# Caltech-OCTO/Subzero.jl

Measured on AMD Instinct MI355X. Metric: floe_steps_per_sec, higher is better.
Workload: dtype f64

## Files before the change

### subzero.jl_amd/csrc/sz_api.hip

```cpp
#include <hip/hip_runtime.h>
#include <dlfcn.h>
#include <execinfo.h>
#include <signal.h>
#include <unistd.h>
#include <algorithm>
#include <cmath>
#include <cstdio>
#include <cstring>
#include <string>
#include <vector>

#include "../../include/subzero_hip.h"
#include "sz_kernels.hpp"
#include "sz_pipeline.hpp"
#include "sz_twoway.hpp"
#include "sz_output.hpp"
#include "sz_migrate.hpp"
#include "sz_fracture.hpp"
#include "sz_weld.hpp"
#include "sz_remove_tile.hpp"
#include "sz_fracture_tile.hpp"
#include "sz_weld_tile.hpp"
#include <rocprim/rocprim.hpp>
#include "sz_ctx.hpp"
// ... 168 lines not shown
  (void)hipMemsetAsync(c->S.cell_ovf, 0, ((size_t)c->S.capCells + 1) * sizeof(int), c->stream);
  hipLaunchKernelGGL(sz_k_cell_build, dim3(grid_for(c->S.capM, 256)), dim3(256), 0, c->stream, c->S, 1);
  c->grid_live = true;
}

void world_rings(sz_ctx* c) {
  if (!c->rings_stale) return;
  hipLaunchKernelGGL(sz_k_world_rings, dim3(grid_for(c->S.capM, 256)), dim3(256), 0, c->stream, c->S);
  c->rings_stale = false;
}
void leave_resident(sz_ctx* c) { c->gl_valid = false; c->S.famrec = 0; c->crec_current = false; world_rings(c); }
struct BatchModes {
  sz_ctx* c;
  explicit BatchModes(sz_ctx* c_) : c(c_) { clear(); }
  ~BatchModes() { clear(); }
  BatchModes(const BatchModes&) = delete;
  BatchModes& operator=(const BatchModes&) = delete;
  void clear() {
    State& S = c->S;
    S.step = 0; S.retry_stop = 0; S.stop_on_tags = 0; S.restart_on_tags = 0; S.ginline = 0; S.famrec = 0; S.body_rings = 0;
    S.crec = nullptr; S.facc = nullptr; S.goff = 0; S.gcap = 0; S.pipe = 0;
    c->acc_mode = 0; c->reduce_mode = 0;
  }
};

void use_ghost_list(sz_ctx* c) {
  if (c->gl_valid) return;
  (void)hipMemsetAsync(c->S.cnt + C_NGCAND, 0, 2 * sizeof(int), c->stream);
  c->gl_cur = 0;
  hipLaunchKernelGGL(sz_k_ghost_seed, dim3(grid_for(c->S.capM, 256)), dim3(256), 0, c->stream, c->S, 0);
  c->gl_valid = true;
}
int reseed_inline_ghosts(sz_ctx* c, int slot) {
  HIPCHK(c, hipMemsetAsync(c->S.galloc, 0, 32 * sizeof(unsigned long long), c->stream));
  c->S.gslot = slot;
  hipLaunchKernelGGL(sz_k_ghost_inline_seed, dim3(grid_for(c->S.capM, 256)), dim3(256), 0, c->stream, c->S, slot, c->hostN);
  return SZ_OK;
}
bool ghost_list_wanted(const sz_ctx* c, bool sg) {
  return sg && !c->no_ghost_list && (c->S.any_periodic_ew || c->S.any_periodic_ns) && c->gl_est <= c->gl_max && c->max_ring <= 64;
}

void stage_ghosts(sz_ctx* c, bool in_step = false, bool commit = false, bool use_list = false) {
  State& S = c->S;
  const int nh = in_step && !S.tiled ? c->hostN : -1;
  if (!S.any_periodic_ew && !S.any_periodic_ns) return;
  S.famrec = in_step ? 1 : 0;
  Timed t(c, SZ_K_GHOSTS);
  if (use_list) {
    const int waves = std::min(std::max(2 * c->gl_est + 64, 256), 8192);
    hipLaunchKernelGGL(sz_k_ghost_list, dim3((waves + 3) / 4), dim3(256), 0, c->stream, S, c->gl_cur, 1, nh);
    t.end();
    return;
  }
  const int nb = grid_for(S.capM, SCAN_B, 1 << 20);
  hipLaunchKernelGGL(sz_k_ghost_flag_scan, dim3(nb), dim3(SCAN_B), 0, c->stream, S, in_step ? 1 : 0, commit ? 1 : 0, next_epoch(c), nh);
  hipLaunchKernelGGL(sz_k_ghost_fill, dim3(grid_for(S.capM, 32, 2048)), dim3(256), 0, c->stream, S, commit ? 1 : 0, commit ? 1 : 0, nh);
  if (!in_step) hipLaunchKernelGGL(sz_k_ghost_commit, dim3(1), dim3(64), 0, c->stream, S);
  t.end();
}

int search_grid(const State& T) { return grid_for(T.capM, NB_TPB / NB_G, 8192); }
void launch_search(sz_ctx* c, const State& T, bool elems = false, bool forcing = false) {
  const bool rec = T.crec != nullptr;
  if (forcing) {
    const int nbn = grid_for(T.capM, 256 / NB_G, 8192), nbf = grid_for(T.capM, 256 / FRC_PLAIN, 8192);
    const auto kern = c->precision == 1 ? (rec ? sz_k_neighbors_forcing<2, true> : sz_k_neighbors_forcing<2, false>)
// ... 569 lines not shown
  std::vector<int> tag0;
  DA(frc_remove, S.capM); DA(osign, S.capM); DA(bbx0, S.capM); DA(bbx1, S.capM); DA(bby0, S.capM); DA(bby1, S.capM);
  {
    std::vector<long long> id(M), gid(M, 0);
    std::vector<int> st(M, SZ_ACTIVE), parent(M), gh((size_t)MAX_GHOSTS * M, -1), ngh(M, 0);
    for (int i = 0; i < M; i++) { id[i] = f->id ? f->id[i] : i + 1; if (f->ghost_id) gid[i] = f->ghost_id[i]; if (f->status) st[i] = f->status[i]; parent[i] = i; }
    if (M > N) {
      for (int i = 0; i < N; i++) {
        int n = f->ghost_off[i + 1] - f->ghost_off[i];
        if (n > MAX_GHOSTS) { c->err = "more than 3 ghosts for one parent"; return SZ_E_ARG; }
        ngh[i] = n;
        for (int k = 0; k < n; k++) { int g = f->ghost_idx[f->ghost_off[i] + k]; if (g < N || g >= M) { c->err = "ghost index out of range"; return SZ_E_ARG; } gh[(size_t)i * MAX_GHOSTS + k] = g; parent[g] = i; }
      }
    }
    { std::vector<long long> ok(S.capM); for (int i = 0; i < S.capM; i++) ok[i] = i; H2D(S.okey, ok.data(), S.capM, long long); HIPCHK(c, hipStreamSynchronize(c->stream)); }
    H2D(S.id, id.data(), M, long long); H2D(S.ghost_id, gid.data(), M, long long); H2D(S.status, st.data(), M, int);
    tag0 = st;
    H2D(S.parent, parent.data(), M, int); H2D(S.gh, gh.data(), (size_t)MAX_GHOSTS * M, int); H2D(S.ngh, ngh.data(), M, int);
    HIPCHK(c, hipStreamSynchronize(c->stream));
  }
  DA(voff, S.capM + 1); DA(vxy, S.capV);
  H2D(S.voff, f->vert_off, M + 1, int);
  {
    std::vector<double> xy((size_t)2 * std::max(V, 1));
    for (int k = 0; k < V; k++) { xy[(size_t)2 * k] = f->vx[k]; xy[(size_t)2 * k + 1] = f->vy[k]; }
    H2D(S.vxy, xy.data(), (size_t)2 * V, double); HIPCHK(c, hipStreamSynchronize(c->stream));
  }
  DA(soff, S.capM + 1); DA(sx, NS); DA(sy, NS);
  if (f->sub_off) { H2D(S.soff, f->sub_off, N + 1, int); H2D(S.sx, f->sx, NS, double); H2D(S.sy, f->sy, NS, double); }
  c->max_sub = 0;
  if (f->sub_off) for (int i = 0; i < N; i++) c->max_sub = std::max(c->max_sub, f->sub_off[i + 1] - f->sub_off[i]);
  DA(gplan, S.capM + 1); DA(gscan4, S.capM + 1); DA(gtot4, 4);
  DA(lb_agg, S.capM / 128 + 8); DA(lb_inc, S.capM / 128 + 8); DA(lb_flag, S.capM / 128 + 8);
  DA(gflag, S.capM + 1); DA(gvscan, S.capM + 2); DA(gcand, (size_t)2 * S.capM); DA(galloc, 32); DA(gkeys, (size_t)2 * S.capM); DA(fam, S.capM);
  DA(crec, (size_t)8 * S.capM); c->crec_buf = S.crec; S.crec = nullptr;
  {
    StepSet& B = c->pb[1];
    if ((rc = dalloc(c, &B.vxy, (size_t)S.capV, c->allocs)) || (rc = dalloc(c, &B.crec, (size_t)8 * S.capM, c->allocs)) ||
        (rc = dalloc(c, &B.gh, (size_t)MAX_GHOSTS * S.capM, c->allocs)) || (rc = dalloc(c, &B.ngh, (size_t)S.capM, c->allocs))) return rc;
    HIPCHK(c, hipMemsetAsync(B.gh, 0xff, (size_t)MAX_GHOSTS * S.capM * sizeof(int), c->stream));
    c->gpar = 0;
  }
  DA(facc, (size_t)FX_WORDS * S.capM); c->facc_buf = S.facc; S.facc = nullptr;
  c->maybe_tagged = false;
  if (f->status) for (int i = 0; i < N; i++) if (f->status[i] != SZ_ACTIVE) { c->maybe_tagged = true; break; }
  for (int k = 0; k < 4; k++) if ((rc = dalloc(c, &c->frc_alt[k], (size_t)S.capM, c->allocs))) return rc;
  DA(bounds, 16 + 64 * 4); DA(cell_cnt, S.capCells + 1); DA(cell_ovf, S.capCells + 1); DA(cell_slots, (size_t)S.capCells * CELL_K + 8);
  DA(cell_items, S.capM);
  {
    StepSet& B = c->pb[1];
    if ((rc = dalloc(c, &B.cell_cnt, (size_t)S.capCells + 1, c->allocs)) || (rc = dalloc(c, &B.cell_ovf, (size_t)S.capCells + 1, c->allocs)) ||
        (rc = dalloc(c, &B.cell_slots, (size_t)S.capCells * CELL_K + 8, c->allocs)) || (rc = dalloc(c, &B.cell_items, (size_t)S.capM, c->allocs))) return rc;
  }
  DA(n_out, S.capM + 1); DA(n_in, S.capM + 1); DA(over_stamp, S.capM + 1); DA(over_base, S.capM + 1);
  DA(out_off, S.capM + 2);
  DA(el_off, S.capM + 2); DA(el_floe, S.capElem); DA(el_elem, S.capElem);
  DA(inter_off, S.capM + 2);
  if (!f->sub_off) HIPCHK(c, hipMemsetAsync(S.soff, 0, ((size_t)S.capM + 1) * sizeof(int), c->stream));
  if ((rc = carve_lists(c))) return rc;
  if ((rc = carve_interactions(c))) return rc;
  DA(blk, std::max(S.capCells, std::max(S.capM, 1024)) / SCAN_B + 1024);
  own_set_carved(c);
  DA(tagA, S.capM + 1);
  if (!tag0.empty()) { H2D(S.tagA, tag0.data(), M, int); HIPCHK(c, hipStreamSynchronize(c->stream)); }
  if ((rc = dalloc(c, &c->origin, (size_t)S.capM, c->allocs))) return rc;
  { std::vector<int> o(std::max(M, 1)); for (int i = 0; i < M; i++) o[i] = i; H2D(c->origin, o.data(), M, int); HIPCHK(c, hipStreamSynchronize(c->stream)); }
  DA(stamps, 512 + 8 * 8000);
  trim_pool(c->allocs);
  free_pool(c->comm_allocs);
  int gl_est = N;
  double rmax_max = 0.0;
  if (f->rmax) {
    const double x0 = c->h_vals[3], xf = c->h_vals[2], y0 = c->h_vals[1], yf = c->h_vals[0];
    const bool pew = c->h_kinds[SZ_EAST] == SZ_PERIODIC && c->h_kinds[SZ_WEST] == SZ_PERIODIC;
    const bool pns = c->h_kinds[SZ_NORTH] == SZ_PERIODIC && c->h_kinds[SZ_SOUTH] == SZ_PERIODIC;
    gl_est = 0;
    for (int i = 0; i < N; i++) {
      const double r = f->rmax[i];
      if ((pew && (f->cx[i] - r < x0 || f->cx[i] + r > xf)) || (pns && (f->cy[i] - r < y0 || f->cy[i] + r > yf))) gl_est++;
    }
// ... 561 lines not shown
  p.pipe = pipeline_eligible(c, p, nsteps, flags);
  p.lean = p.coll && lean_wanted(c) && (p.pipe || !c->S.tiled);
  p.first_alone = p.rfree && c->maybe_tagged && p.user_stop && nsteps > 1;
  p.frac = c->frac_kind != SZ_FRAC_OFF && p.user_stop && !p.pipe;
  return p;
}

int step_batch_pipelined(sz_ctx* c, const BatchPlan& plan, int nsteps, int tstep0, int dt, int coupling_dt, int flags, int* h, int* done_out, int* slot_out, bool* rest_out) {
  State& S0 = c->S;
  const int N = c->hostN;
  const bool fam = N <= 40000 && plan.periodic;
  const bool elems = S0.any_domain_work != 0;
  const int q0 = c->gpar;
  auto par = [&](int s) { return (q0 + s) & 1; };
  S0.restart_on_tags = plan.user_stop ? 0 : 1;
  bool lean = plan.lean;
  Clears clr(c);
  clr.add(c->facc_buf, (size_t)FX_WORDS * S0.capM * sizeof(long long));
  clr.add(S0.cnt + C_FRCSTOP, sizeof(int));
  const int callid0 = c->callid; c->callid += nsteps;
  bool first_start = true;
  auto prologue = [&](int s) {
    const int q = par(s);
    pipe_adopt(c, q);
    S0.step = 0; S0.goff = 0; S0.gcap = 0;
    if (!first_start) c->grid_live = false;
    use_static_grid(c);
    const StepSet& O = c->pb[1 - q];
    clr.add(O.cell_cnt, ((size_t)S0.capCells + 1) * sizeof(int));
    clr.add(O.cell_ovf, ((size_t)S0.capCells + 1) * sizeof(int));
    clr.add(c->pb[0].wq, NSEG * 32 * sizeof(int)); clr.add(c->pb[1].wq, NSEG * 32 * sizeof(int));
    clr.add(c->pb[0].ngh, (size_t)S0.capM * sizeof(int));
    clr.add(c->pb[1].ngh, (size_t)S0.capM * sizeof(int));
    clr.add(S0.galloc, 32 * sizeof(unsigned long long));
    clr.launch(c);
    if (!(first_start && c->crec_current))
      for (int b = 0; b < 2; b++) { State T = pipe_state(c, b); T.step = 0; seed_records(c, T, N); }
    first_start = false;
    State T = pipe_state(c, q); T.step = s + 1; T.callid = callid0 + s + 1; T.retry_stop = lean ? 1 : 0;
    if (plan.gi) hipLaunchKernelGGL(sz_k_ghost_inline_seed, dim3(grid_for(S0.capM, 256)), dim3(256), 0, c->stream, T, q, N);
    launch_search(c, T, elems);
  };
  auto launch_L1 = [&](int s, bool make_ghosts) {
    State T = pipe_state(c, par(s)); T.step = s + 1; T.callid = callid0 + s + 1; T.retry_stop = lean ? 1 : 0;
    const PipeAlt A = pipe_alt(c, par(s + 1), make_ghosts ? 1 : 0);
    const bool coupling = coupling_at(flags, coupling_dt, tstep0 + s);
    const bool overlap = coupling && (c->overlap_forcing >= 0 ? c->overlap_forcing != 0 : N > 65536);
    if (overlap) stage_forcing_fork(c, &T);
    if (coupling) c->forcing_where = overlap ? 0 : 2;
    const bool frc = coupling && !overlap;
    launch_narrow_first(c, frc ? narrow_first<1, 1> : narrow_first<0, 1>, T, dt, c->P.ff_max_overlap, c->P.fd_max_overlap, frc, &A, N);
    if (!lean) narrow_largest(c, T, dt, c->P.ff_max_overlap, c->P.fd_max_overlap, 256);
    return overlap;
  };
  auto launch_L2 = [&](int s, bool with_search, bool host_last, bool joined) {
    if (joined) stage_forcing_join(c);
    State T = pipe_state(c, par(s + 1)); T.step = s + 2; T.callid = callid0 + s + 2; T.retry_stop = lean ? 1 : 0;
    const PipeAlt A = pipe_alt(c, par(s), 0);
    const int nbv = grid_for(N, NB_TPB, 1 << 20), nbs = with_search ? search_grid(T) : 0;
    const int nbe = with_search && elems ? grid_for(N, NB_TPB, 1 << 20) : 0;
    const unsigned ep = nbe ? next_epoch(c) : 0u;
    const int am = 1 | 4 | (host_last ? 2 : 0);
    Timed tm(c, SZ_K_INTEGRATE);
    if (fam) hipLaunchKernelGGL((sz_k_vel_search<true>), dim3(nbv + nbs + nbe), dim3(NB_TPB), 0, c->stream, T, c->P, A, dt, coupling_at(flags, coupling_dt, tstep0 + s) ? 1 : 0, nbv, N, am, nbe, ep);
    else hipLaunchKernelGGL((sz_k_vel_search<false>), dim3(nbv + nbs + nbe), dim3(NB_TPB), 0, c->stream, T, c->P, A, dt, coupling_at(flags, coupling_dt, tstep0 + s) ? 1 : 0, nbv, N, am, nbe, ep);
    tm.end();
  };
// ... 902 lines not shown
```

### subzero.jl_amd/csrc/sz_kernels.hpp

```cpp
#pragma once
#include <type_traits>
#include "sz_geom.hpp"
#include "sz_state.hpp"

namespace sz {
using namespace szg;

#define SZ_ACTIVE 1
#define SZ_REMOVE 2
#define SZ_FUSE 3

__device__ __forceinline__ bool stopped(const State& S) {
  const int s = S.cnt[C_STOP], r = S.cnt[C_RETRYSTOP];
  return (s != 0 && S.step > s) || (r != 0 && S.step > r);
}
__device__ __forceinline__ bool stopped_late(const State& S) {
  const int s = S.cnt[C_STOP], r = S.cnt[C_RETRYSTOP];
  return (s != 0 && S.step > s) || (r != 0 && S.step >= r);
}
struct StopRegs { int s, r; };
__device__ __forceinline__ StopRegs stop_load(const State& S) { StopRegs q; q.s = S.cnt[C_STOP]; q.r = S.cnt[C_RETRYSTOP]; return q; }
__device__ __forceinline__ bool stop_test(const State& S, const StopRegs& q) { return (q.s != 0 && S.step > q.s) || (q.r != 0 && S.step > q.r); }
__device__ __forceinline__ bool stop_test_late(const State& S, const StopRegs& q) { return (q.s != 0 && S.step > q.s) || (q.r != 0 && S.step >= q.r); }
__device__ __forceinline__ void loads_issued() { asm volatile("" ::: "memory"); }
__device__ __forceinline__ void request_stop(const State& S) {
  if (S.step > 0 && S.stop_on_tags) S.cnt[C_STOP] = S.step;
}
__device__ __forceinline__ void request_stop_new_tag(const State& S) {
  if (S.step > 0 && (S.stop_on_tags || S.restart_on_tags)) S.cnt[C_STOP] = S.step;
}
__device__ __forceinline__ void capacity_stop(const State& S) {
  if (S.step > 0) S.cnt[C_RETRYSTOP] = S.step;
}

__device__ __forceinline__ int ring_off(const State& S, int i) { return S.body_rings ? S.rb_off[i] : S.voff[i]; }
__device__ __forceinline__ int ring_n(const State& S, int i) { return S.body_rings ? S.rb_n[i] : S.voff[i + 1] - S.voff[i]; }
constexpr float MIX_CIRCLE_MARGIN = 4.0f, MIX_BOX_MARGIN = 2.0f;
__device__ __forceinline__ void rec32_store(const State& S, int i, double cx, double cy, double r, double x0, double x1, double y0, double y1) {
  S.rec32[2 * (size_t)i] = make_float4((float)cx, (float)cy, (float)r, 0.0f);
  S.rec32[2 * (size_t)i + 1] = make_float4((float)x0, (float)x1, (float)y0, (float)y1);
}

constexpr long long CREC_KEYMASK = (1ll << 48) - 1;
__device__ __forceinline__ double crec_okf(long long okey, int nv, int osign) {
  return __longlong_as_double(okey | ((long long)(nv & 255) << 48) | ((long long)(osign < 0 ? 1 : 0) << 56));
}
__device__ __forceinline__ double crec_vp(int voff, int parent, int ngh) {
  return __longlong_as_double((long long)(unsigned)voff | ((long long)parent << 32) | ((long long)ngh << 60));
}
__device__ __forceinline__ void crec_store_all(const State& S, int row, double cx, double cy, double rmax, long long id, long long okey, int nv, int osign,
                                               int voff, int parent, int ngh, double x0, double x1, double y0, double y1, double u, double v, double xi,
                                               double area, double h, long long ghost_id) {
  double2* r = S.crec + (size_t)row * 8;
  r[0] = make_double2(cx, cy); r[1] = make_double2(rmax, __longlong_as_double(id));
  r[2] = make_double2(crec_okf(okey, nv, osign), crec_vp(voff, parent, ngh));
  r[3] = make_double2(x0, x1); r[4] = make_double2(y0, y1); r[5] = make_double2(u, v); r[6] = make_double2(xi, area);
  r[7] = make_double2(h, __longlong_as_double(ghost_id));
// ... 930 lines not shown
    return idx < cnt ? start + idx : -1;
  }
  const int q = nblk / 8, r = nblk % 8;
  return (x < r ? x * (q + 1) : r * (q + 1) + (x - r) * q) + idx;
}


struct Seg { int s, np, ne, n; };
__device__ __forceinline__ int seg_cap(const State& S) { return S.capPairs / NSEG; }
__device__ __forceinline__ Seg seg_of(const State& S, int s) {
  Seg g; g.s = s; g.np = S.wq[s * 32 + 1];
  const int nel = S.cnt[C_NELEM];
  g.ne = nel > s ? (nel - s + NSEG - 1) / NSEG : 0;
  g.n = g.np + g.ne;
  return g;
}
struct Item { int i, j, e, rows, info, ao, na, bo, nb; bool is_pair; };
__device__ __forceinline__ Item item_of(const State& S, const Seg& g, int t) {
  Item it; it.is_pair = t < g.np;
  if (it.is_pair) {
    const int w = g.s * seg_cap(S) + t;
    const int4 k = S.work[2 * (size_t)w], r = S.work[2 * (size_t)w + 1];
    it.info = k.x; it.i = k.y; it.j = k.z; it.e = -1; it.rows = w; it.ao = k.w; it.na = r.x; it.bo = r.y; it.nb = r.z;
  } else {
    const int q = (t - g.np) * NSEG + g.s; it.i = S.el_floe[q]; it.e = S.el_elem[q]; it.j = -1; it.rows = S.capPairs + q; it.info = S.capM * S.maxnb + q;
    it.ao = ring_off(S, it.i); it.na = ring_n(S, it.i); it.bo = S.eoff[it.e]; it.nb = S.eoff[it.e + 1] - it.bo;
  }
  return it;
}

constexpr int NB_G = 16, NB_TPB = 128;
static_assert(NB_G == FX_WORDS, "the neighbour search clears a new row's fixed-point totals with one store per lane");
template <int TPB, bool FAM = true, int NBC = MAXNB, bool REC = false>
__device__ __forceinline__ void neighbors_body(State& S, int bid, int nblk) {
  constexpr int GPB = TPB / NB_G;
  constexpr int NB_POOL = NBC <= 24 ? 96 : (NBC <= 64 ? 224 : 256);
  constexpr int MW = (NBC + 63) / 64;
  static_assert(NB_POOL >= NBC, "the pool is reused for the sorted list of the owned pairs");
  __shared__ int cand[GPB][2][NBC];
  __shared__ long long ckey[GPB][2][NBC];
  __shared__ int cnts[GPB][2];
  using mask_t = typename std::conditional<(NBC <= 32), unsigned, unsigned long long>::type;
  __shared__ mask_t wmask[MW > 1 ? 1 : GPB];
  __shared__ unsigned long long wmaskw[MW > 1 ? GPB : 1][MW];
  __shared__ int pool[GPB][NB_POOL];
  __shared__ int pool2[GPB][NBC > MAXNB ? NB_POOL : 1];
  __shared__ int npool[GPB];
  __shared__ int wbase[GPB + 1];
  __shared__ int cvo[GPB][NBC], cnv[GPB][NBC], svo[GPB][NBC], snv[GPB][NBC];
  __shared__ double kbox[REC ? GPB : 1][4];
  const int gl = threadIdx.x % NB_G, gi = threadIdx.x / NB_G;
  const StopRegs stop = stop_load(S);
  int M = S.cnt[C_M];
  int nfix = 0x7fffffff;
  int nsplit = 0x7fffffff, kshift = 0, lim0 = M, lim1 = M;
  if (S.ginline) {
    const unsigned long long a = S.galloc[S.gslot * 16], poisoned = S.galloc[S.gslot * 16 + 1];
    const int N = S.cnt[C_N]; int G = (int)(a >> 32), V = (int)(a & 0xffffffffull);
    if (REC && S.facc) nfix = N;
    if (poisoned || N + S.goff + G > S.capM || (S.gcap > 0 && G > S.gcap)) { G = 0; V = 0; }
    M = N + G; lim0 = M; lim1 = M;
    if (bid == 0 && threadIdx.x == 0 && !stop_test(S, stop)) { S.cnt[C_M] = M; S.cnt[C_NV] = S.voff[N] + V; S.cnt[C_NGHOSTS] = G; }
    if (REC && S.goff != 0) { nsplit = (N + 15) & ~15; kshift = N + S.goff - nsplit; lim0 = N; lim1 = N + S.goff + G; M = nsplit + G; }
  }
  const GridGeo g = grid_geo(S);
  const int ncx = g.ncx, ncy = g.ncy;
  const int seg = bid % NSEG, segcap = seg_cap(S);
  static_assert(16 % GPB == 0 || GPB % 16 == 0, "blocks of rows must not straddle nsplit");
  for (int kb = bid * GPB; kb < S.capM; kb += nblk * GPB) {
    const bool hi = REC && kb >= nsplit;
    const int k = (hi ? kb + kshift : kb) + gi;
    const bool act = k < (hi ? lim1 : lim0);
    double ckx = 0, cky = 0, rk = 0, kx0 = 0, kx1 = 0, ky0 = 0, ky1 = 0;
    long long idk = 0, okk = 0, kgid = 0; bool kplain = true; int ix = 0, iy = 0, vok = 0, nvk = 0, kpar = 0;
    if (k < S.capM) {
      if constexpr (REC) {
        const double2* rr = S.crec + (size_t)k * 8;
        const double2 q0 = rr[0], q1 = rr[1], q2 = rr[2], q3 = rr[3], q4 = rr[4];
        const long long okf = __double_as_longlong(q2.x), vp = __double_as_longlong(q2.y);
        ckx = q0.x; cky = q0.y; rk = q1.x; idk = __double_as_longlong(q1.y);
        okk = okf & CREC_KEYMASK; nvk = (int)(okf >> 48) & 255; vok = (int)(unsigned)vp;
        kpar = (int)(vp >> 32) & 0x0fffffff; kplain = kpar == k && (vp >> 60) == 0;
        if (gl == 0) { kbox[gi][0] = q3.x; kbox[gi][1] = q3.y; kbox[gi][2] = q4.x; kbox[gi][3] = q4.y; }
      } else {
        vok = ring_off(S, k); nvk = ring_n(S, k);
        ckx = S.cx[k]; cky = S.cy[k]; rk = S.rmax[k];
        kx0 = S.bbx0[k]; kx1 = S.bbx1[k]; ky0 = S.bby0[k]; ky1 = S.bby1[k];
        idk = S.id[k]; okk = S.okey[k];
        kpar = S.parent[k]; kplain = kpar == k && S.ngh[k] == 0; kgid = S.ghost_id[k];
      }
    }
    loads_issued();
    if (stop_test(S, stop) || kb >= M) break;
    if (bid == 0 && threadIdx.x == 0 && kb == bid * GPB) { S.cnt[C_ITEMCLASS] = 0; S.cnt[C_NFUSE] = 0; }
    if constexpr (REC) { if (act && k >= nfix) S.facc[(size_t)k * FX_WORDS + gl] = 0; }
    __syncthreads();
    if (gl == 0) { cnts[gi][0] = 0; cnts[gi][1] = 0; npool[gi] = 0; if constexpr (MW == 1) wmask[gi] = (mask_t)0; }
    if constexpr (MW > 1) { if (gl < MW) wmaskw[gi][gl] = 0ull; }
    __syncthreads();
    if (act) cell_of(g, ckx, cky, ix, iy);
    bool ovf = false;
    auto candidates = [&](int np) {
      for (int e = gl; e < np; e += NB_G) {
        int o;
        if constexpr (NBC > MAXNB) o = pool2[gi][e]; else o = pool[gi][e];
        if (o == k) continue;
        if (S.rec32) {
          const float4 oc = S.rec32[2 * (size_t)o];
          const float fdx = (float)ckx - oc.x, fdy = (float)cky - oc.y;
          const float frr = (float)rk + oc.z + MIX_CIRCLE_MARGIN + 1e-6f * fmaxf(fabsf((float)ckx), fabsf((float)cky));
          if (!(fdx * fdx + fdy * fdy < frr * frr)) continue;
        }
        double ocx, ocy, orm, ox0, ox1, oy0, oy1; long long oid, ko; int opar, voo, nvo; bool oplain;
        if constexpr (REC) {
          const double2* ro = S.crec + (size_t)o * 8;
          const double2 q0 = ro[0], q1 = ro[1], q2 = ro[2], q3 = ro[3], q4 = ro[4];
          const long long okf = __double_as_longlong(q2.x), vp = __double_as_longlong(q2.y);
          ocx = q0.x; ocy = q0.y; orm = q1.x; oid = __double_as_longlong(q1.y);
          ko = okf & CREC_KEYMASK; nvo = (int)(okf >> 48) & 255; voo = (int)(unsigned)vp;
          opar = (int)(vp >> 32) & 0x0fffffff; oplain = opar == o && (vp >> 60) == 0;
          ox0 = q3.x; ox1 = q3.y; oy0 = q4.x; oy1 = q4.y;
        } else {
          ocx = S.cx[o]; ocy = S.cy[o]; orm = S.rmax[o];
// ... 246 lines not shown
  if (o + c > S.capElem) return;
  elem_candidates<REC>(S, k, [&](int e) { S.el_floe[o] = k; S.el_elem[o] = e; o++; });
}
__global__ void __launch_bounds__(SCAN_B) sz_k_elem_scan_fill(State S, unsigned epoch) { elem_scan_fill_body(S, epoch, (int)blockIdx.x); }
template <bool FAM, bool REC = false>
__global__ void __launch_bounds__(NB_TPB) sz_k_neighbors_elem(State S, unsigned epoch, int nbn) {
  if ((int)blockIdx.x < nbn) neighbors_body<NB_TPB, FAM, MAXNB, REC>(S, blockIdx.x, nbn);
  else elem_scan_fill_body(S, epoch, (int)blockIdx.x - nbn);
}

template <bool TW>
__device__ __forceinline__ void forcing_body(State& S, const Params& P, int bid, int nblk, int pmax);
__device__ __forceinline__ void forcing_mixed_body(State& S, const Params& P, int bid, int nblk);
__device__ __forceinline__ void geo_body(State S, const PipeAlt& A, int dt, int bid, int nblk, int N);
template <int G, int CAP, int KC, int RC, int RM, int TPB, int LO, int CLS, int WPE = 1, int FRC = 0, int GEO = 0>
__global__ void __launch_bounds__(TPB, WPE) sz_k_narrow(State S, Params P, int dt, double ff_max_overlap, double fd_max_overlap, int dbg, int nbf,
                                                       PipeAlt PA, int nbg, int nn) {
  constexpr int GPB = TPB / G;
  const int nblk = (int)gridDim.x - (FRC != 0 ? nbf : 0) - (GEO != 0 ? nbg : 0);
  if (GEO != 0 && (int)blockIdx.x < nbg) { geo_body(S, PA, dt, (int)blockIdx.x, nbg, nn); return; }
  const int bidx = (int)blockIdx.x - (GEO != 0 ? nbg : 0);
  if (FRC != 0 && bidx >= nblk) {
    if (FRC == 1) forcing_body<false>(S, P, bidx - nblk, nbf, 0);
    else forcing_mixed_body(S, P, bidx - nblk, nbf);
    return;
  }
  static_assert(4 * KC <= 2 * RC, "raw crossing slots alias reg[1]");
  Stamps st; STAMP_INIT(st);
#ifdef SZ_STAMPS
  st.on = (CLS == 0 && bidx == (dbg >> 8) && threadIdx.x == 0); st.log = S.stamps + 1;
#endif
  const int qk = bidx % NSEG;
  const int t_first = (bidx / NSEG) * (TPB / G) + (int)(threadIdx.x / G);
  const bool pre_ok = !(G == 64 && TPB == 64) && t_first < seg_cap(S);
  int4 pre0 = make_int4(0, 0, 0, 0), pre1 = make_int4(0, 0, 0, 0);
  if (pre_ok) { const size_t w2 = 2 * ((size_t)qk * seg_cap(S) + t_first); pre0 = S.work[w2]; pre1 = S.work[w2 + 1]; }
  const StopRegs stop = stop_load(S);
  const Seg sg = seg_of(S, qk);
  const int icls = CLS > 0 ? S.cnt[C_ITEMCLASS] : 0;
  loads_issued();
  if (CLS > 0 && icls < CLS) return;
  if (stop_test(S, stop)) return;
  STAMP(st, 20);
  __shared__ GroupMem<CAP, KC, RC, RM> mem[GPB];
  const int gl = threadIdx.x % G, gi = threadIdx.x / G;
  GroupMem<CAP, KC, RC, RM>& m = mem[gi];
  const int nitems = sg.n;
  if (gl == 0) { m.err = 0; m.ierr = 0; m.ntracefail = 0; m.nchk = 0; m.nkeep = 0; m.acc[0] = m.acc[1] = 0; m.acc16[0] = m.acc16[1] = m.acc16[2] = m.acc16[3] = m.acc16[4] = 0; }
  if (CLS == 0) {
    const int ncells = (int)S.bounds[4] * (int)S.bounds[5];
    for (int q = bidx * TPB + threadIdx.x; q <= ncells; q += nblk * TPB) { S.cell_cnt[q] = 0; S.cell_ovf[q] = 0; }
    if (bidx == 0) for (int q = threadIdx.x; q < WARN_SLOTS * 4; q += TPB) S.warn[(q >> 2) * 32 + (q & 3)] = 0;
    if (S.ginline && !GEO && bidx == 0 && threadIdx.x == 0) { S.galloc[(1 - S.gslot) * 16] = 0ull; S.galloc[(1 - S.gslot) * 16 + 1] = 0ull; }
    if (bidx == 0 && threadIdx.x == 0 && (S.cnt[C_ERR] & (ERR_CAP_NEIGH | ERR_CAP_PAIRS))) capacity_stop(S);
  }
  STAMP(st, 21);
  constexpr bool SCAN = (G == 64 && TPB == 64);
  constexpr int STRIDE = SCAN ? 64 : GPB;
  const bool useq = CLS == 0 && !SCAN;
  const int rb = bidx / NSEG, nbq = (nblk + NSEG - 1 - qk) / NSEG;
  const int limit = nitems;
  for (int t0 = rb * STRIDE; t0 < limit;) {
   unsigned long long todo = 1;
   int tk_next = 0;
   if (SCAN) {
     const int tt = t0 + (int)threadIdx.x;
     bool want = false;
     if (tt < nitems) {
       const Item it_ = item_of(S, sg, tt);
       const int nb_ = it_.nb, na_ = it_.na;
       want = (na_ > nb_ ? na_ : nb_) > LO || ((S.it_info[it_.info].x >> 8) & IT_RETRY);
     }
     todo = __ballot(want);
   }
   while (todo) {
#ifdef SZ_STAMPS
    st.tmark = clock64();
    if (st.cP < 0) st.cP = st.tmark - st.t0w;
#endif
    int t;
    if (SCAN) { t = t0 + __ffsll((long long)todo) - 1; todo &= todo - 1; }
    else { todo = 0; t = t0 + gi; }
    bool have = t < limit;
    Item it; it.i = 0; it.j = -1; it.e = -1; it.rows = 0; it.info = 0; it.is_pair = true; it.ao = it.na = it.bo = it.nb = 0;
    if (have) {
      if (pre_ok && t == t_first && t < sg.np) {
        it.is_pair = true; it.info = pre0.x; it.i = pre0.y; it.j = pre0.z; it.e = -1; it.rows = qk * seg_cap(S) + t;
// ... 1689 lines not shown
```

### subzero.jl_amd/csrc/sz_pipeline.hpp

```cpp
#pragma once
#include "sz_kernels.hpp"

namespace sz {

__device__ __forceinline__ State pipe_other(State S, const PipeAlt& A) {
  step_set_copy(S, A); S.goff = A.goff; S.gslot = A.gslot;
  return S;
}

struct GhostRowLite { double cx, cy, b0, b1, b2, b3, rmax, area, h, mass, mom, al, u, v, xi, over, tc, ts; long long id, oki; int st; signed char os; };
struct RingMoved {
  const double2* src; double cx, cy, dx, dy, cda, sda;
  __device__ __forceinline__ void get(int k, double& mx, double& my) const {
    const double2 p = src[k];
    const double x = p.x + (-cx), y = p.y + (-cy);
    const double xr = cda * x - sda * y, yr = sda * x + cda * y;
    mx = xr + (cx + dx); my = yr + (cy + dy);
  }
};
__device__ __forceinline__ void geo_body(State S, const PipeAlt& A, int dt, int bid, int nblk, int N) {
  const StopRegs stop = stop_load(S);
  State So = pipe_other(S, A);
  So.pipe = 1;
  const GridGeo geo = grid_geo(S);
// ... 28 lines not shown
      if (cell_s < CELL_K) So.cell_slots[(size_t)cell_c * CELL_K + cell_s] = i;
      else So.cell_items[i] = atomicExch(&So.cell_ovf[cell_c], i + 1) - 1;
#pragma unroll
      for (int k = 0; k < MV_RING; k++) {
        if (k < n) {
          const double x = p[k].x + (-cx), y = p[k].y + (-cy);
          const double xr = cda * x - sda * y, yr = sda * x + cda * y;
          const double mx = xr + (cx + dx), my = yr + (cy + dy);
          So.vxy[o + k] = make_double2(mx, my);
          bx0 = fmin(bx0, mx); bx1 = fmax(bx1, mx); by0 = fmin(by0, my); by1 = fmax(by1, my);
        }
      }
    }
    {
      double2* r = So.crec + (size_t)i * 8;
      r[0] = make_double2(ncx, ncy); r[2].y = crec_vp(o, i, 0); r[3] = make_double2(bx0, bx1); r[4] = make_double2(by0, by1);
    }
    const int gf = A.make_ghosts ? ghost_flag_of(wall, S.any_periodic_ew, S.any_periodic_ns, ncx, ncy, rmx, bx0, bx1, by0, by1, st0 == SZ_ACTIVE) : 5;
    if (gf != 5) {
      GhostRowLite R;
      R.cx = ncx; R.cy = ncy; R.b0 = bx0; R.b1 = bx1; R.b2 = by0; R.b3 = by1;
      R.rmax = rmx; R.area = S.area[i]; R.h = S.height[i]; R.mass = 0.0; R.mom = 0.0; R.al = 0.0; R.u = u; R.v = v; R.xi = xi;
      R.over = S.overarea[i]; R.id = S.id[i]; R.oki = S.okey[i]; R.os = S.osign[i]; R.st = SZ_ACTIVE; R.tc = 1.0; R.ts = 0.0;
      const RingMoved ring{ S.vxy + o, cx, cy, dx, dy, cda, sda };
      ghost_inline_make(So, geo, wall, N, nv0, A.gslot, i, gf, n, o, R, ring);
    } else {
      So.ngh[i] = 0;
    }
  }
}

__device__ __forceinline__ void vel_body(State S, const Params& P, const PipeAlt& A, int dt, int apply_frc, int bid, int nblk, int N, int acc_mode) {
  const int step = S.step - 1;
  const int cs = S.cnt[C_STOP], cr = S.cnt[C_RETRYSTOP], frcstop = S.cnt[C_FRCSTOP];
  const bool halted = (cs != 0 && step > cs) || (cr != 0 && step >= cr);
  const bool last_step = (acc_mode & 2) != 0 || ((S.stop_on_tags || S.restart_on_tags) && (cs == step || frcstop == step));
  if (bid == 0 && !halted) {
    if (threadIdx.x < 2 * NSEG) A.wq[(threadIdx.x >> 1) * 32 + (threadIdx.x & 1)] = 0;
    if (threadIdx.x == 0) { S.galloc[(1 - S.gslot) * 16] = 0ull; S.galloc[(1 - S.gslot) * 16 + 1] = 0ull; }
  }
  int wh = 0, wf = 0, wv = 0, wx = 0;
  bool tested = false;
  for (int i = bid * (int)blockDim.x + (int)threadIdx.x; i < N; i += nblk * (int)blockDim.x) {
    const int st0 = S.status[i], ngh0 = A.ngh[i] & 0xff;
    const double rmx = S.rmax[i], area = S.area[i], height0 = S.height[i];
    longlong4 fa0, fa1, fa2, fa3;
    { const longlong4* a = (const longlong4*)(S.facc + (size_t)i * FX_WORDS); fa0 = a[0]; fa1 = a[1]; fa2 = a[2]; fa3 = a[3]; }
    double g_over = S.overarea[i];
    const int frc_rm = apply_frc ? S.frc_remove[i] : 0;
    if (!tested) {
      loads_issued();
      if (halted) break;
      tested = true;
    }
    double cfx, cfy, ctrq, s11 = 0, s12 = 0, s21 = 0, s22 = 0;
    int st_new = st0; bool st_dirty = false;
    {
      long long q[7] = { fa0.x, fa0.y, fa0.z, fa0.w, fa1.x, fa1.y, fa1.z }, ql[7] = { fa2.x, fa2.y, fa2.z, fa2.w, fa3.x, fa3.y, fa3.z };
      const int tagb = (int)(fa1.w & 0xffffffffll);
      const bool dirty = (fa0.x | fa0.y | fa0.z | fa0.w | fa1.x | fa1.y | fa1.z | fa1.w | fa2.x | fa2.y | fa2.z | fa2.w | fa3.x | fa3.y | fa3.z) != 0;
      if (ngh0 != 0) {
        for (int g3i = 0; g3i < MAX_GHOSTS; g3i++) {
          const int g = A.gh[i * MAX_GHOSTS + g3i];
          if (g >= 0) {
            const longlong4* a = (const longlong4*)(S.facc + (size_t)g * FX_WORDS); const longlong4 b0 = a[0], b1 = a[1], b2 = a[2], b3 = a[3];
            q[0] += b0.x; q[1] += b0.y; q[2] += b0.z; q[3] += b0.w; q[4] += b1.x; q[5] += b1.y; q[6] += b1.z;
            ql[0] += b2.x; ql[1] += b2.y; ql[2] += b2.z; ql[3] += b2.w; ql[4] += b3.x; ql[5] += b3.y; ql[6] += b3.z;
// ... 66 lines not shown
    const int ngh1 = S.ngh[i];
    const double cx = S.cx[i], cy = S.cy[i];
    double2* r = S.crec + (size_t)i * 8;
    const double2 g0 = r[0], g3 = r[3], g4 = r[4];
    if (last_step) {
      double cda, sda;
      sincos(da, &sda, &cda);
      *(double4*)(S.mot + (size_t)i * 4) = make_double4(cx, cy, 1.5 * dt * u - 0.5 * dt * p_dxdt, 1.5 * dt * v - 0.5 * dt * p_dydt);
      *(double2*)(S.mot2 + (size_t)i * 2) = make_double2(cda, sda);
    }
    S.cx[i] = g0.x; S.cy[i] = g0.y; S.bbx0[i] = g3.x; S.bbx1[i] = g3.y; S.bby0[i] = g4.x; S.bby1[i] = g4.y;
    r[5] = make_double2(nu, nv); r[6] = make_double2(nxi, area); r[7].x = h;
    for (int q = 0; q < (ngh1 & 0xff); q++) {
      const int g = S.gh[i * MAX_GHOSTS + q];
      if (g < 0) continue;
      double2* rg = S.crec + (size_t)g * 8;
      rg[5] = make_double2(nu, nv); rg[6] = make_double2(nxi, area); rg[7].x = h;
      S.u[g] = nu; S.v[g] = nv; S.xi[g] = nxi; S.height[g] = h; S.overarea[g] = g_over;
    }
  }
  for (int d = 32; d >= 1; d >>= 1) { wh += __shfl_xor(wh, d); wf += __shfl_xor(wf, d); wv += __shfl_xor(wv, d); wx += __shfl_xor(wx, d); }
  if ((threadIdx.x & 63) == 0) {
    int* w = S.warn + (((bid * blockDim.x + threadIdx.x) >> 6) % WARN_SLOTS) * 32;
    if (wh) atomicAdd(w + 0, wh);
    if (wf) atomicAdd(w + 1, wf);
    if (wv) atomicAdd(w + 2, wv);
    if (wx) atomicAdd(w + 3, wx);
  }
}

template <bool FAM>
__global__ void __launch_bounds__(NB_TPB, 3) sz_k_vel_search(State S, Params P, PipeAlt A, int dt, int apply_frc, int nbv, int N, int acc_mode, int nbe, unsigned epoch) {
  if ((int)blockIdx.x < nbv) { vel_body(S, P, A, dt, apply_frc, (int)blockIdx.x, nbv, N, acc_mode); return; }
  if ((S.stop_on_tags || S.restart_on_tags) && S.cnt[C_FRCSTOP] == S.step - 1 && S.step > 1) return;
  const int nbs = (int)gridDim.x - nbv - nbe;
  if ((int)blockIdx.x < nbv + nbs) neighbors_body<NB_TPB, FAM, MAXNB, true>(S, (int)blockIdx.x - nbv, nbs);
  else elem_scan_fill_body<true>(S, epoch, (int)blockIdx.x - nbv - nbs, N);
}

__global__ void __launch_bounds__(128) sz_k_unswap(State S, PipeAlt A, int N) {
  for (int i = blockIdx.x * blockDim.x + threadIdx.x; i < N; i += gridDim.x * blockDim.x) {
    if (!(S.ngh[i] & 0x100)) continue;
    const double4 m = *(const double4*)(S.mot + (size_t)i * 4);
    const double2 t = *(const double2*)(S.mot2 + (size_t)i * 2);
    const double cx = m.x, cy = m.y, dx = m.z, dy = m.w, cda = t.x, sda = t.y;
    const int o = S.voff[i], n = S.voff[i + 1] - o;
    double bx0 = __builtin_inf(), bx1 = -__builtin_inf(), by0 = __builtin_inf(), by1 = -__builtin_inf();
    for (int k = 0; k < n; k++) {
      const double2 p = A.vxy[o + k];
      const double x = p.x + (-cx), y = p.y + (-cy);
      const double xr = cda * x - sda * y, yr = sda * x + cda * y;
      const double mx = xr + (cx + dx), my = yr + (cy + dy);
      S.vxy[o + k] = make_double2(mx, my);
      bx0 = fmin(bx0, mx); bx1 = fmax(bx1, mx); by0 = fmin(by0, my); by1 = fmax(by1, my);
    }
    const double ncx = cx + dx, ncy = cy + dy;
    S.cx[i] = ncx; S.cy[i] = ncy; S.bbx0[i] = bx0; S.bbx1[i] = bx1; S.bby0[i] = by0; S.bby1[i] = by1;
    double2* r = S.crec + (size_t)i * 8;
    r[0] = make_double2(ncx, ncy); r[3] = make_double2(bx0, bx1); r[4] = make_double2(by0, by1);
  }
}

__global__ void __launch_bounds__(256) sz_k_rows_home(State S, int N, int G, int goff) {
  const int nb = S.maxnb, M = N + G;
  for (long long t = (long long)blockIdx.x * blockDim.x + threadIdx.x; t < (long long)G * nb; t += (long long)gridDim.x * blockDim.x) {
    const int g = (int)(t / nb), e = (int)(t % nb);
    const size_t src = (size_t)(N + goff + g) * nb + e, dst = (size_t)(N + g) * nb + e;
    S.nb_out[dst] = S.nb_out[src]; S.nb_in[dst] = S.nb_in[src]; S.it_info[dst] = S.it_info[src];
    if (e == 0) {
      const int a = N + goff + g, b = N + g;
// ... 21 lines not shown
```

### subzero.jl_amd/csrc/sz_state.hpp

```cpp
#pragma once
#include <hip/hip_runtime.h>
#include <stdint.h>

namespace sz {

enum {
  C_M = 0,
  C_N,
  C_NV,
  C_NPAIRS,
  C_NELEM,
  C_NINTER,
  C_ERR,
  C_NPAIR_PTS,
  C_NPAIR_ROWS,
  C_NELEM_ROWS,
  C_NGCAND, C_NGCAND1,
  C_NFUSE,
  C_RETRYSTOP,
  C_NG_NEW,
  C_NGHOSTS,
  C_NCELLS,
  C_SCRATCH0, C_SCRATCH1,
  C_TRACE_FAIL,
  C_NOWN,
  C_NHALO,
  C_ITEMCLASS,
  C_NRETRY,
  C_NWORK,
  C_NENT,
  C_STOP,
  C_DRIFT,
  C_PAUSED,
  C_FRCSTOP,
  C_COUNT = 32
};

constexpr int MAXNB = 24;
constexpr int CELL_K = 8;
constexpr int NSEG = 8;
constexpr int ROWS_PER_ITEM = 16;
constexpr int WARN_SLOTS = 256;
constexpr int ACC_SLOTS = 256;
constexpr int MAX_GHOSTS = 3;

struct Params {
  double E, nu, mu, rho_o, rho_a, Cd_io, Cd_ia, fcor, turn;
  double ff_max_overlap, fd_max_overlap;
  double rho_i, max_h, max_xi, lambda;
  int dd;
  double Cd_ao, k_ice, L_ice;
};

struct State {
  int capM, capV, capPairs, capElem, capRows, capCells, capS;
  int nelem;
  int any_periodic_ew, any_periodic_ns, any_domain_work;
  int tiled;
  int step;
  int retry_stop;
  int stop_on_tags;
  int goff;
  int halo_ring;
  int gcap;
  int pipe;
  int restart_on_tags;
  int* cnt;
  int* warn;
  double *cx, *cy, *rmax, *area, *height, *mass, *moment, *alpha, *u, *v, *xi;
  double *p_dxdt, *p_dydt, *p_dalphadt, *p_dudt, *p_dvdt, *p_dxidt;
  double *fxOA, *fyOA, *trqOA, *hflx, *overarea, *cfx, *cfy, *ctrq;
  double *sa, *si, *strain;
  long long *id, *ghost_id, *okey;
  int *status, *parent, *gh, *ngh, *frc_remove;
  int *gh_save, *ngh_save;
  signed char* osign;
  double *bbx0, *bbx1, *bby0, *bby1;
// ... 67 lines not shown
```

Measured before the change: 129.4 million.

## Batch kernel-front control reads into one wave-wide load with readlane broadcast

Kernel prologues for the neighbour search, narrow-phase items and velocity step now issue one vector load per lane covering the control counters, plus galloc, bounds or segment words, and extract scalars via readlane instead of several dependent scalar loads. The neighbour search also speculatively prefetches its first record before the stop and M checks, and the FRCSTOP gate moves into the search body so those loads overlap. This aims to cut serialized load latency at kernel start, at the cost of more complex code and wasted loads when the kernel exits early.

```diff
diff --git a/subzero.jl_amd/csrc/sz_api.hip b/subzero.jl_amd/csrc/sz_api.hip
--- a/subzero.jl_amd/csrc/sz_api.hip
+++ b/subzero.jl_amd/csrc/sz_api.hip
@@ -224,7 +224,7 @@
   c->gl_valid = true;
 }
 int reseed_inline_ghosts(sz_ctx* c, int slot) {
-  HIPCHK(c, hipMemsetAsync(c->S.galloc, 0, 32 * sizeof(unsigned long long), c->stream));
+  HIPCHK(c, hipMemsetAsync(c->S.galloc, 0, GALLOC_WORDS * sizeof(unsigned long long), c->stream));
   c->S.gslot = slot;
   hipLaunchKernelGGL(sz_k_ghost_inline_seed, dim3(grid_for(c->S.capM, 256)), dim3(256), 0, c->stream, c->S, slot, c->hostN);
   return SZ_OK;
@@ -860,7 +860,7 @@
   if (f->sub_off) for (int i = 0; i < N; i++) c->max_sub = std::max(c->max_sub, f->sub_off[i + 1] - f->sub_off[i]);
   DA(gplan, S.capM + 1); DA(gscan4, S.capM + 1); DA(gtot4, 4);
   DA(lb_agg, S.capM / 128 + 8); DA(lb_inc, S.capM / 128 + 8); DA(lb_flag, S.capM / 128 + 8);
-  DA(gflag, S.capM + 1); DA(gvscan, S.capM + 2); DA(gcand, (size_t)2 * S.capM); DA(galloc, 32); DA(gkeys, (size_t)2 * S.capM); DA(fam, S.capM);
+  DA(gflag, S.capM + 1); DA(gvscan, S.capM + 2); DA(gcand, (size_t)2 * S.capM); DA(galloc, GALLOC_WORDS); DA(gkeys, (size_t)2 * S.capM); DA(fam, S.capM);
   DA(crec, (size_t)8 * S.capM); c->crec_buf = S.crec; S.crec = nullptr;
   {
     StepSet& B = c->pb[1];
@@ -873,7 +873,7 @@
   c->maybe_tagged = false;
   if (f->status) for (int i = 0; i < N; i++) if (f->status[i] != SZ_ACTIVE) { c->maybe_tagged = true; break; }
   for (int k = 0; k < 4; k++) if ((rc = dalloc(c, &c->frc_alt[k], (size_t)S.capM, c->allocs))) return rc;
-  DA(bounds, 16 + 64 * 4); DA(cell_cnt, S.capCells + 1); DA(cell_ovf, S.capCells + 1); DA(cell_slots, (size_t)S.capCells * CELL_K + 8);
+  DA(bounds, BOUNDS_WORDS); DA(cell_cnt, S.capCells + 1); DA(cell_ovf, S.capCells + 1); DA(cell_slots, (size_t)S.capCells * CELL_K + 8);
   DA(cell_items, S.capM);
   {
     StepSet& B = c->pb[1];
@@ -1501,7 +1501,7 @@
     clr.add(c->pb[0].wq, NSEG * 32 * sizeof(int)); clr.add(c->pb[1].wq, NSEG * 32 * sizeof(int));
     clr.add(c->pb[0].ngh, (size_t)S0.capM * sizeof(int));
     clr.add(c->pb[1].ngh, (size_t)S0.capM * sizeof(int));
-    clr.add(S0.galloc, 32 * sizeof(unsigned long long));
+    clr.add(S0.galloc, GALLOC_WORDS * sizeof(unsigned long long));
     clr.launch(c);
     if (!(first_start && c->crec_current))
       for (int b = 0; b < 2; b++) { State T = pipe_state(c, b); T.step = 0; seed_records(c, T, N); }
diff --git a/subzero.jl_amd/csrc/sz_kernels.hpp b/subzero.jl_amd/csrc/sz_kernels.hpp
--- a/subzero.jl_amd/csrc/sz_kernels.hpp
+++ b/subzero.jl_amd/csrc/sz_kernels.hpp
@@ -23,6 +23,31 @@
 __device__ __forceinline__ bool stop_test(const State& S, const StopRegs& q) { return (q.s != 0 && S.step > q.s) || (q.r != 0 && S.step > q.r); }
 __device__ __forceinline__ bool stop_test_late(const State& S, const StopRegs& q) { return (q.s != 0 && S.step > q.s) || (q.r != 0 && S.step >= q.r); }
 __device__ __forceinline__ void loads_issued() { asm volatile("" ::: "memory"); }
+constexpr int FRONT_CNT = 32, FRONT_X = 8;
+static_assert(FRONT_CNT <= C_COUNT && (FRONT_CNT & (FRONT_CNT - 1)) == 0, "the front reads cnt[0 .. FRONT_CNT)");
+static_assert(C_STOP < FRONT_CNT && C_RETRYSTOP < FRONT_CNT && C_FRCSTOP < FRONT_CNT && C_ITEMCLASS < FRONT_CNT, "control words of the fronts");
+static_assert(16 + 2 <= GALLOC_WORDS && 4 + 2 <= BOUNDS_WORDS, "the fronts read galloc[gslot * 16 + {0, 1}] and bounds[4 .. 5]");
+typedef int __attribute__((may_alias)) front_dword;
+struct FrontRegs { int c, x; };
+__device__ __forceinline__ FrontRegs front_issue(const State& S, const front_dword* xp) {
+  FrontRegs f; f.c = S.cnt[threadIdx.x & (FRONT_CNT - 1)]; f.x = *xp; return f;
+}
+__device__ __forceinline__ void front_wait(FrontRegs& f) { asm volatile("" : "+v"(f.c), "+v"(f.x) : : "memory"); }
+__device__ __forceinline__ int front_word(int v, int lane) { return __builtin_amdgcn_readlane(v, lane); }
+__device__ __forceinline__ unsigned long long front_word64(int v, int lane) {
+  return (unsigned long long)(unsigned)front_word(v, lane) | (unsigned long long)(unsigned)front_word(v, lane + 1) << 32;
+}
+__device__ __forceinline__ StopRegs front_stop(const FrontRegs& f) { StopRegs q; q.s = front_word(f.c, C_STOP); q.r = front_word(f.c, C_RETRYSTOP); return q; }
+__device__ __forceinline__ const front_dword* front_x_narrow(const State& S, int seg, bool cells) {
+  const int l = (int)(threadIdx.x & (FRONT_X - 1));
+  const front_dword* p = (const front_dword*)(S.wq + seg * 32 + 1);
+  if (cells && l >= 1 && l <= 4) p = (const front_dword*)(S.bounds + 4) + (l - 1);
+  return p;
+}
+__device__ __forceinline__ const front_dword* front_x_search(const State& S) {
+  const int l = (int)(threadIdx.x & 3);
+  return (S.ginline ? (const front_dword*)(S.galloc + S.gslot * 16) : (const front_dword*)S.cnt) + l;
+}
 __device__ __forceinline__ void request_stop(const State& S) {
   if (S.step > 0 && S.stop_on_tags) S.cnt[C_STOP] = S.step;
 }
@@ -1019,7 +1044,7 @@
 constexpr int NB_G = 16, NB_TPB = 128;
 static_assert(NB_G == FX_WORDS, "the neighbour search clears a new row's fixed-point totals with one store per lane");
 template <int TPB, bool FAM = true, int NBC = MAXNB, bool REC = false>
-__device__ __forceinline__ void neighbors_body(State& S, int bid, int nblk) {
+__device__ __forceinline__ void neighbors_body(State& S, int bid, int nblk, int Nh = -1, bool frc_gate = false) {
   constexpr int GPB = TPB / NB_G;
   constexpr int NB_POOL = NBC <= 24 ? 96 : (NBC <= 64 ? 224 : 256);
   constexpr int MW = (NBC + 63) / 64;
@@ -1037,45 +1062,62 @@
   __shared__ int cvo[GPB][NBC], cnv[GPB][NBC], svo[GPB][NBC], snv[GPB][NBC];
   __shared__ double kbox[REC ? GPB : 1][4];
   const int gl = threadIdx.x % NB_G, gi = threadIdx.x / NB_G;
-  const StopRegs stop = stop_load(S);
-  int M = S.cnt[C_M];
+  FrontRegs fr = front_issue(S, front_x_search(S));
+  const GridGeo g = grid_geo(S);
+  const int ncx = g.ncx, ncy = g.ncy;
+  const bool split = REC && S.ginline && S.goff != 0;
+  int kbase_spec = bid * GPB;
+  if (split) {
+    const int ns = (Nh + 15) & ~15;
+    kbase_spec = Nh < 0 ? -1 : kbase_spec >= ns ? kbase_spec + (Nh + S.goff - ns) : kbase_spec;
+  }
+  double2 q0 = make_double2(0, 0), q1 = q0, q2 = q0, q3 = q0, q4 = q0;
+  auto own_record = [&](int kbase) {
+    if constexpr (REC) {
+      const int kr = kbase + gi < S.capM ? (kbase + gi < 0 ? 0 : kbase + gi) : S.capM - 1;
+      const double2* rr = S.crec + (size_t)kr * 8;
+      q0 = rr[0]; q1 = rr[1]; q2 = rr[2]; q3 = rr[3]; q4 = rr[4];
+    }
+  };
+  own_record(kbase_spec);
+  front_wait(fr);
+  const StopRegs stop = front_stop(fr);
+  if (frc_gate && (S.stop_on_tags || S.restart_on_tags) && S.step > 1 && front_word(fr.c, C_FRCSTOP) == S.step - 1) return;
+  int M = front_word(fr.c, C_M);
   int nfix = 0x7fffffff;
   int nsplit = 0x7fffffff, kshift = 0, lim0 = M, lim1 = M;
   if (S.ginline) {
-    const unsigned long long a = S.galloc[S.gslot * 16], poisoned = S.galloc[S.gslot * 16 + 1];
-    const int N = S.cnt[C_N]; int G = (int)(a >> 32), V = (int)(a & 0xffffffffull);
+    const unsigned long long a = front_word64(fr.x, 0), poisoned = front_word64(fr.x, 2);
+    const int N = front_word(fr.c, C_N); int G = (int)(a >> 32), V = (int)(a & 0xffffffffull);
     if (REC && S.facc) nfix = N;
     if (poisoned || N + S.goff + G > S.capM || (S.gcap > 0 && G > S.gcap)) { G = 0; V = 0; }
     M = N + G; lim0 = M; lim1 = M;
     if (bid == 0 && threadIdx.x == 0 && !stop_test(S, stop)) { S.cnt[C_M] = M; S.cnt[C_NV] = S.voff[N] + V; S.cnt[C_NGHOSTS] = G; }
     if (REC && S.goff != 0) { nsplit = (N + 15) & ~15; kshift = N + S.goff - nsplit; lim0 = N; lim1 = N + S.goff + G; M = nsplit + G; }
   }
-  const GridGeo g = grid_geo(S);
-  const int ncx = g.ncx, ncy = g.ncy;
   const int seg = bid % NSEG, segcap = seg_cap(S);
   static_assert(16 % GPB == 0 || GPB % 16 == 0, "blocks of rows must not straddle nsplit");
-  for (int kb = bid * GPB; kb < S.capM; kb += nblk * GPB) {
+  const int kstride = nblk * GPB;
+  auto kbase_of = [&](int kb) { return REC && kb >= nsplit ? kb + kshift : kb; };
+  if (REC && kbase_of(bid * GPB) != kbase_spec) own_record(kbase_of(bid * GPB));
+  for (int kb = bid * GPB; kb < S.capM; kb += kstride, (REC && kb < S.capM ? own_record(kbase_of(kb)) : (void)0)) {
     const bool hi = REC && kb >= nsplit;
-    const int k = (hi ? kb + kshift : kb) + gi;
+    const int k = kbase_of(kb) + gi;
     const bool act = k < (hi ? lim1 : lim0);
     double ckx = 0, cky = 0, rk = 0, kx0 = 0, kx1 = 0, ky0 = 0, ky1 = 0;
     long long idk = 0, okk = 0, kgid = 0; bool kplain = true; int ix = 0, iy = 0, vok = 0, nvk = 0, kpar = 0;
-    if (k < S.capM) {
-      if constexpr (REC) {
-        const double2* rr = S.crec + (size_t)k * 8;
-        const double2 q0 = rr[0], q1 = rr[1], q2 = rr[2], q3 = rr[3], q4 = rr[4];
-        const long long okf = __double_as_longlong(q2.x), vp = __double_as_longlong(q2.y);
-        ckx = q0.x; cky = q0.y; rk = q1.x; idk = __double_as_longlong(q1.y);
-        okk = okf & CREC_KEYMASK; nvk = (int)(okf >> 48) & 255; vok = (int)(unsigned)vp;
-        kpar = (int)(vp >> 32) & 0x0fffffff; kplain = kpar == k && (vp >> 60) == 0;
-        if (gl == 0) { kbox[gi][0] = q3.x; kbox[gi][1] = q3.y; kbox[gi][2] = q4.x; kbox[gi][3] = q4.y; }
-      } else {
-        vok = ring_off(S, k); nvk = ring_n(S, k);
-        ckx = S.cx[k]; cky = S.cy[k]; rk = S.rmax[k];
-        kx0 = S.bbx0[k]; kx1 = S.bbx1[k]; ky0 = S.bby0[k]; ky1 = S.bby1[k];
-        idk = S.id[k]; okk = S.okey[k];
-        kpar = S.parent[k]; kplain = kpar == k && S.ngh[k] == 0; kgid = S.ghost_id[k];
-      }
+    if constexpr (REC) {
+      const long long okf = __double_as_longlong(q2.x), vp = __double_as_longlong(q2.y);
+      ckx = q0.x; cky = q0.y; rk = q1.x; idk = __double_as_longlong(q1.y);
+      okk = okf & CREC_KEYMASK; nvk = (int)(okf >> 48) & 255; vok = (int)(unsigned)vp;
+      kpar = (int)(vp >> 32) & 0x0fffffff; kplain = kpar == k && (vp >> 60) == 0;
+      if (gl == 0) { kbox[gi][0] = q3.x; kbox[gi][1] = q3.y; kbox[gi][2] = q4.x; kbox[gi][3] = q4.y; }
+    } else if (k < S.capM) {
+      vok = ring_off(S, k); nvk = ring_n(S, k);
+      ckx = S.cx[k]; cky = S.cy[k]; rk = S.rmax[k];
+      kx0 = S.bbx0[k]; kx1 = S.bbx1[k]; ky0 = S.bby0[k]; ky1 = S.bby1[k];
+      idk = S.id[k]; okk = S.okey[k];
+      kpar = S.parent[k]; kplain = kpar == k && S.ngh[k] == 0; kgid = S.ghost_id[k];
     }
     loads_issued();
     if (stop_test(S, stop) || kb >= M) break;
@@ -1388,27 +1430,32 @@
 #endif
   const int qk = bidx % NSEG;
   const int t_first = (bidx / NSEG) * (TPB / G) + (int)(threadIdx.x / G);
-  const bool pre_ok = !(G == 64 && TPB == 64) && t_first < seg_cap(S);
+  constexpr bool PRE = !(G == 64 && TPB == 64);
+  const bool pre_ok = PRE && t_first < seg_cap(S);
+  FrontRegs fr = front_issue(S, front_x_narrow(S, qk, CLS == 0));
   int4 pre0 = make_int4(0, 0, 0, 0), pre1 = make_int4(0, 0, 0, 0);
-  if (pre_ok) { const size_t w2 = 2 * ((size_t)qk * seg_cap(S) + t_first); pre0 = S.work[w2]; pre1 = S.work[w2 + 1]; }
-  const StopRegs stop = stop_load(S);
-  const Seg sg = seg_of(S, qk);
-  const int icls = CLS > 0 ? S.cnt[C_ITEMCLASS] : 0;
-  loads_issued();
+  if constexpr (PRE) {
+    const size_t w2 = 2 * ((size_t)qk * seg_cap(S) + (pre_ok ? t_first : 0)); pre0 = S.work[w2]; pre1 = S.work[w2 + 1];
+  }
+  __shared__ GroupMem<CAP, KC, RC, RM> mem[GPB];
+  const int gl = threadIdx.x % G, gi = threadIdx.x / G;
+  GroupMem<CAP, KC, RC, RM>& m = mem[gi];
+  if (gl == 0) { m.err = 0; m.ierr = 0; m.ntracefail = 0; m.nchk = 0; m.nkeep = 0; m.acc[0] = m.acc[1] = 0; m.acc16[0] = m.acc16[1] = m.acc16[2] = m.acc16[3] = m.acc16[4] = 0; }
+  front_wait(fr);
+  const StopRegs stop = front_stop(fr);
+  Seg sg; sg.s = qk; sg.np = front_word(fr.x, 0);
+  { const int nel = front_word(fr.c, C_NELEM); sg.ne = nel > qk ? (nel - qk + NSEG - 1) / NSEG : 0; sg.n = sg.np + sg.ne; }
+  const int icls = CLS > 0 ? front_word(fr.c, C_ITEMCLASS) : 0;
   if (CLS > 0 && icls < CLS) return;
   if (stop_test(S, stop)) return;
   STAMP(st, 20);
-  __shared__ GroupMem<CAP, KC, RC, RM> mem[GPB];
-  const int gl = threadIdx.x % G, gi = threadIdx.x / G;
-  GroupMem<CAP, KC, RC, RM>& m = mem[gi];
   const int nitems = sg.n;
-  if (gl == 0) { m.err = 0; m.ierr = 0; m.ntracefail = 0; m.nchk = 0; m.nkeep = 0; m.acc[0] = m.acc[1] = 0; m.acc16[0] = m.acc16[1] = m.acc16[2] = m.acc16[3] = m.acc16[4] = 0; }
   if (CLS == 0) {
-    const int ncells = (int)S.bounds[4] * (int)S.bounds[5];
+    const int ncells = (int)__hiloint2double(front_word(fr.x, 2), front_word(fr.x, 1)) * (int)__hiloint2double(front_word(fr.x, 4), front_word(fr.x, 3));
     for (int q = bidx * TPB + threadIdx.x; q <= ncells; q += nblk * TPB) { S.cell_cnt[q] = 0; S.cell_ovf[q] = 0; }
     if (bidx == 0) for (int q = threadIdx.x; q < WARN_SLOTS * 4; q += TPB) S.warn[(q >> 2) * 32 + (q & 3)] = 0;
     if (S.ginline && !GEO && bidx == 0 && threadIdx.x == 0) { S.galloc[(1 - S.gslot) * 16] = 0ull; S.galloc[(1 - S.gslot) * 16 + 1] = 0ull; }
-    if (bidx == 0 && threadIdx.x == 0 && (S.cnt[C_ERR] & (ERR_CAP_NEIGH | ERR_CAP_PAIRS))) capacity_stop(S);
+    if (bidx == 0 && threadIdx.x == 0 && (front_word(fr.c, C_ERR) & (ERR_CAP_NEIGH | ERR_CAP_PAIRS))) capacity_stop(S);
   }
   STAMP(st, 21);
   constexpr bool SCAN = (G == 64 && TPB == 64);
diff --git a/subzero.jl_amd/csrc/sz_pipeline.hpp b/subzero.jl_amd/csrc/sz_pipeline.hpp
--- a/subzero.jl_amd/csrc/sz_pipeline.hpp
+++ b/subzero.jl_amd/csrc/sz_pipeline.hpp
@@ -84,7 +84,9 @@
 
 __device__ __forceinline__ void vel_body(State S, const Params& P, const PipeAlt& A, int dt, int apply_frc, int bid, int nblk, int N, int acc_mode) {
   const int step = S.step - 1;
-  const int cs = S.cnt[C_STOP], cr = S.cnt[C_RETRYSTOP], frcstop = S.cnt[C_FRCSTOP];
+  FrontRegs fr = front_issue(S, (const front_dword*)S.cnt);
+  front_wait(fr);
+  const int cs = front_word(fr.c, C_STOP), cr = front_word(fr.c, C_RETRYSTOP), frcstop = front_word(fr.c, C_FRCSTOP);
   const bool halted = (cs != 0 && step > cs) || (cr != 0 && step >= cr);
   const bool last_step = (acc_mode & 2) != 0 || ((S.stop_on_tags || S.restart_on_tags) && (cs == step || frcstop == step));
   if (bid == 0 && !halted) {
@@ -217,10 +219,10 @@
 template <bool FAM>
 __global__ void __launch_bounds__(NB_TPB, 3) sz_k_vel_search(State S, Params P, PipeAlt A, int dt, int apply_frc, int nbv, int N, int acc_mode, int nbe, unsigned epoch) {
   if ((int)blockIdx.x < nbv) { vel_body(S, P, A, dt, apply_frc, (int)blockIdx.x, nbv, N, acc_mode); return; }
+  const int nbs = (int)gridDim.x - nbv - nbe;
+  if ((int)blockIdx.x < nbv + nbs) { neighbors_body<NB_TPB, FAM, MAXNB, true>(S, (int)blockIdx.x - nbv, nbs, N, true); return; }
   if ((S.stop_on_tags || S.restart_on_tags) && S.cnt[C_FRCSTOP] == S.step - 1 && S.step > 1) return;
-  const int nbs = (int)gridDim.x - nbv - nbe;
-  if ((int)blockIdx.x < nbv + nbs) neighbors_body<NB_TPB, FAM, MAXNB, true>(S, (int)blockIdx.x - nbv, nbs);
-  else elem_scan_fill_body<true>(S, epoch, (int)blockIdx.x - nbv - nbs, N);
+  elem_scan_fill_body<true>(S, epoch, (int)blockIdx.x - nbv - nbs, N);
 }
 
 __global__ void __launch_bounds__(128) sz_k_unswap(State S, PipeAlt A, int N) {
diff --git a/subzero.jl_amd/csrc/sz_state.hpp b/subzero.jl_amd/csrc/sz_state.hpp
--- a/subzero.jl_amd/csrc/sz_state.hpp
+++ b/subzero.jl_amd/csrc/sz_state.hpp
@@ -43,6 +43,8 @@
 constexpr int WARN_SLOTS = 256;
 constexpr int ACC_SLOTS = 256;
 constexpr int MAX_GHOSTS = 3;
+constexpr int GALLOC_WORDS = 32;
+constexpr int BOUNDS_WORDS = 16 + 64 * 4;
 
 struct Params {
   double E, nu, mu, rho_o, rho_a, Cd_io, Cd_ia, fcor, turn;
```

New measurement: 130.6 million, median of 4. About the same (+0.9%).
